# KlrShaK/opencv-SimpleSLAM

Hardware: AMD Instinct MI355X
Metric: frames/sec ALIKED+LightGlue @1241x376 (higher is better)
Workload: dtype f32 (contractions: f16 hi/lo split operands, f32 accumulate; 3 MFMA per product, 2 in attention's P.V = precision 'f16x3p1', the default since r05: profiles/r05_flip_soak.md, r06_flip_soak.md); 1 GPU; C2/C4: synthetic 1241x376x3 uint8 frame stream, ALIKED-n16 extract + LightGlue match (t-1,t), 2048 kpts/frame, min_conf 0.7, random-init weights; inputs resident in HBM before the timed region, features and matches left on the device (the `pcie` leg times the same pipeline with per-round H2D of the frames and D2H of {count, pairs}); max_kpts=2048, lightglue_layers_executed=9, pairs_per_lightglue_launch=8, frames_per_aliked_launch=8

## Files before the change

### opencv-simpleslam_amd/csrc/al_plan.hpp

```cpp
#pragma once
#include <algorithm>
#include <cstddef>
#include <cstdio>

namespace sslam {

constexpr int AL_LONG_SIDE = 1024;
constexpr int AL_PAD_DIV = 32;
constexpr int MAX_FRAMES = 16;
constexpr int B1_SW = 30;
constexpr int B2_SW = 30;
constexpr int DCN3_CS = 1;
constexpr int DCN4_CS = 4;
constexpr int AGG_PRE = 13;
constexpr int ST_W = 32, ST_H = 8;
constexpr int PRE_LDS_MAX = 48 * 1024;
constexpr int NHALO = 10;
constexpr int NW_R = 48, NW_OW = 64 - 2 * NHALO, NW_OH = NW_R - 2 * NHALO;
constexpr int HBINS = 4096;
constexpr int COLLECT_PPT = 16;
constexpr int SEL_CAP = 8192;
constexpr int EDGE_CAP = 2048;
constexpr int CAND_CAP = 1024 * 1024;
constexpr int REFINE_KPB = 32;
constexpr int SDDH_KSPLIT = 4;

constexpr int al_cdiv(int a, int b) { return (a + b - 1) / b; }

struct Dims {
    int H, W, C;
    int h, w;
    int Hp, Wp;
    int pl, pt;
};

enum class ALAggTile { T64x64, T64x128 };

struct ALPlan {
    int F, KF;
    int blur, ky, kx;
    float sy, sx;
    Dims d;
    int to_float_gx, pad_gx;
    int b1_strips, b1_nblk, b1_hs, b1_nb;
    int b2_strips, b2_nblk, b2_hs, b2_nb, b2_waves, b2_gx;
    int H2, W2, HW2, H3, W3, HW3, H4, W4, HW4;
    int pool3_gx, pool4_gx;
    int off3_gx, dcn3_gx, off4_gx, dcn4_gx;
// ... 82 lines not shown
enum class ALRefusal { None, Size, Frames, Blur };
inline ALRefusal al_refusal(const ALPlan& p, int Hp_cap, int Wp_cap, int max_frames, char* msg, size_t n) {
    const Dims& d = p.d;
    if (!(d.Hp <= Hp_cap && d.Wp <= Wp_cap && d.h >= 8 && d.w >= 8)) {
        snprintf(msg, n, "sslam_aliked: network size %dx%d outside the instance capacity %dx%d", d.Hp, d.Wp, Hp_cap, Wp_cap);
        return ALRefusal::Size;
    }
    if (!(p.F >= 1 && p.F <= max_frames)) {
        snprintf(msg, n, "sslam_aliked: %d frames, instance capacity %d", p.F, max_frames);
        return ALRefusal::Frames;
    }
    if (!(p.kx <= 31 && p.ky <= 31)) {
        snprintf(msg, n, "sslam_aliked: blur kernel too large (%d,%d)", p.kx, p.ky);
        return ALRefusal::Blur;
    }
    return ALRefusal::None;
}

struct ALKptPlan {
    int NK;
    int refine_gx, patch_gx, offsets_gx, sample_gx, finalize_gx;
    int rows_x16, rows64, rows64_x16;
    size_t plane;
};

inline ALKptPlan al_kpt_plan(int NK) {
    ALKptPlan k{};
    k.NK = NK;
    k.refine_gx = al_cdiv(NK, REFINE_KPB);
    k.patch_gx = al_cdiv(NK * 3, 4);
    k.rows64 = al_cdiv(NK, 64);
    k.offsets_gx = al_cdiv(NK * 32, 256);
    k.sample_gx = al_cdiv(NK * 16, 4);
    k.rows_x16 = NK * 16;
    k.rows64_x16 = al_cdiv(NK * 16, 64);
    k.finalize_gx = al_cdiv(NK, 4);
    k.plane = (size_t)(NK * 16 + 64) * 128;
    return k;
}

struct ALExtents {
    size_t ctrl, in_u8, fsrc, img, x1, x2, p3, off, t3, x3, p3cl, t3cl, p4cl, t4cl, p4, t4, x4, g2, g3, g4, g2cl, g3cl, g4cl;
    size_t s8, rnorm, g1cl, pre2, pre3, pre4, score, nms, bsum, cand, hist, kp_index, sel_keys;
    size_t kp_norm, kp_score, patch, h32, pos, sampled, feats, raw, out_xy, out_desc, out_score, out_n;
};

inline ALExtents al_extents(size_t HWp, size_t HWi, size_t NK) {
    ALExtents e{};
    e.ctrl = 1;
    e.in_u8 = HWi * 4;
    e.fsrc = 3 * HWi; e.img = 3 * HWp;
    e.x1 = 16 * HWp; e.x2 = 32 * HWp / 4;
    e.p3 = 32 * HWp / 64; e.off = 18 * HWp / 64;
    e.t3 = 64 * HWp / 64; e.x3 = 64 * HWp / 64;
    e.p3cl = 32 * HWp / 64; e.t3cl = 64 * HWp / 64;
    e.p4cl = 64 * HWp / 1024; e.t4cl = 128 * HWp / 1024;
    e.p4 = 64 * HWp / 1024; e.t4 = 128 * HWp / 1024; e.x4 = 128 * HWp / 1024;
    e.g2 = 32 * HWp / 4; e.g3 = 32 * HWp / 64; e.g4 = 32 * HWp / 1024;
    e.g2cl = 32 * HWp / 4; e.g3cl = 32 * HWp / 64; e.g4cl = 32 * HWp / 1024;
    e.s8 = 8 * HWp; e.rnorm = HWp; e.g1cl = 32 * HWp;
// ... 15 lines not shown
```

### opencv-simpleslam_amd/csrc/aliked_kernels.hip

```cpp
#include "common.hpp"
#include "al_plan.hpp"
#include "gemm_f32.hpp"
#include <type_traits>
#include "gemm_f16x3.hpp"

namespace {

using sslam::f32x16;
using sslam::acc_row;
using sslam::GemmSmem;
using sslam::GemmA;
using sslam::gemm_mainloop;
using sslam::Dims;
using sslam::MAX_FRAMES; using sslam::B1_SW; using sslam::B2_SW; using sslam::DCN3_CS; using sslam::DCN4_CS; using sslam::AGG_PRE;
using sslam::ST_W; using sslam::ST_H; using sslam::NHALO; using sslam::NW_R; using sslam::NW_OW; using sslam::NW_OH; using sslam::HBINS;
using sslam::COLLECT_PPT; using sslam::SEL_CAP; using sslam::EDGE_CAP; using sslam::REFINE_KPB; using sslam::SDDH_KSPLIT;

constexpr float SELU_SCALE = 1.0507009873554804934193349852946f;
constexpr float SELU_ALPHA = 1.6732632423543772848170429916717f;
__device__ __forceinline__ float selu(float x) {
    return SELU_SCALE * (x > 0.0f ? x : SELU_ALPHA * (__expf(x) - 1.0f));
}

__device__ __forceinline__ float selu_precise(float x) {
    return SELU_SCALE * (x > 0.0f ? x : SELU_ALPHA * expm1f(x));
}

struct ALCtrl {
    int n_cand;
    int n_kp;
    int overflow;
    int found;
    int range_overflow;
    int pad[11];
};

__device__ __forceinline__ void al_range_note(float amax, ALCtrl* ctrl) {
    if (amax >= 65520.0f && amax < INFINITY) ctrl->range_overflow = 1;
}
// ... 834 lines not shown
    float sy2, sx2, sy8, sx8, sy32, sx32;
    const float *g2cl, *g3cl, *g4cl;
    const float *pre2, *pre3, *pre4;
};

__device__ __forceinline__ Pyr pyr_at(Pyr P, int f, size_t fs) {
    P.x1 = fsh(P.x1, f, fs); P.g2 = fsh(P.g2, f, fs); P.g3 = fsh(P.g3, f, fs); P.g4 = fsh(P.g4, f, fs);
    P.g1cl = fsh(P.g1cl, f, fs); P.g2cl = fsh(P.g2cl, f, fs); P.g3cl = fsh(P.g3cl, f, fs); P.g4cl = fsh(P.g4cl, f, fs);
    P.pre2 = fsh(P.pre2, f, fs); P.pre3 = fsh(P.pre3, f, fs); P.pre4 = fsh(P.pre4, f, fs);
    return P;
}

struct UpTap { int o00, o01, o10, o11; float w00, w01, w10, w11; };

__device__ __forceinline__ UpTap up_tap(int y, int x, int Hp, int Wp, int S, float sy, float sx) {
    const int ih = Hp / S, iw = Wp / S;
    const float fy = sy * (float)y, fx = sx * (float)x;
    const int y0 = (int)fy, x0 = (int)fx;
    const int y1 = y0 + (y0 < ih - 1), x1 = x0 + (x0 < iw - 1);
    const float ly = fy - (float)y0, lx = fx - (float)x0, hy = 1.0f - ly, hx = 1.0f - lx;
    UpTap t;
    t.o00 = y0 * iw + x0; t.o01 = y0 * iw + x1; t.o10 = y1 * iw + x0; t.o11 = y1 * iw + x1;
    t.w00 = hx; t.w01 = lx; t.w10 = hy; t.w11 = ly;
    return t;
}
__device__ __forceinline__ float up_eval_cl(const float* __restrict__ p, const UpTap& t, int c) {
    return t.w10 * (t.w00 * p[t.o00 * 32 + c] + t.w01 * p[t.o01 * 32 + c]) +
           t.w11 * (t.w00 * p[t.o10 * 32 + c] + t.w01 * p[t.o11 * 32 + c]);
}
__device__ __forceinline__ float up_eval(const float* __restrict__ p, const UpTap& t) {
    return t.w10 * (t.w00 * p[t.o00] + t.w01 * p[t.o01]) + t.w11 * (t.w00 * p[t.o10] + t.w01 * p[t.o11]);
}

constexpr int PRE_UNROLL = 32;
__global__ __launch_bounds__(256) void al_agg_pre_kernel(const float* __restrict__ g2cl , const float* __restrict__ g3cl,
                                                         const float* __restrict__ g4cl, const float* __restrict__ ws0 ,
                                                         float* __restrict__ pre2, float* __restrict__ pre3, float* __restrict__ pre4,
                                                         int Hp, int Wp, size_t fs) {
    const int f = blockIdx.y;
    const int n2 = (Hp / 2) * (Wp / 2), n3 = (Hp / 8) * (Wp / 8), n4 = (Hp / 32) * (Wp / 32);
    int i = blockIdx.x * blockDim.x + threadIdx.x;
    const float* g; float* pre; int S, lvl;
    if (i < n2) { g = g2cl; pre = pre2; S = 2; lvl = 1; }
    else if (i < n2 + n3) { i -= n2; g = g3cl; pre = pre3; S = 8; lvl = 2; }
    else if (i < n2 + n3 + n4) { i -= n2 + n3; g = g4cl; pre = pre4; S = 32; lvl = 3; }
    else return;
// ... 608 lines not shown
    rnorm = fsh(rnorm, blockIdx.y, fs); kp_norm = fsh(kp_norm, blockIdx.y, fs); patch = fsh(patch, blockIdx.y, fs);
    ctrl = fsh(ctrl, blockIdx.y, fs);
    const int lane = threadIdx.x & 63, gw = blockIdx.x * 4 + __builtin_amdgcn_readfirstlane(threadIdx.x >> 6);
    const int n = gw / 3, trow = gw % 3;
    if (n >= ctrl->n_kp) return;
    const float kx = (kp_norm[2 * n] / 2.0f + 0.5f) * (float)(w - 1);
    const float ky = (kp_norm[2 * n + 1] / 2.0f + 0.5f) * (float)(h - 1);
    int cx = (int)((float)(int)kx - 1.5f + 1.0f), cy = (int)((float)(int)ky - 1.5f + 1.0f);
    cx = min(max(cx, 0), w - 1 - 3);
    cy = min(max(cy, 0), h - 1 - 3);
    float2 f[3];
#pragma unroll
    for (int tc = 0; tc < 3; ++tc) f[tc] = feat_pair32(P, rnorm, pl, pt, cy + trow, cx + tc, lane);
    const int c = lane & 31;
    const int ca = lane < 32 ? c : 32 + c, cb = lane < 32 ? 64 + c : 96 + c;
    float* dst = patch + (size_t)n * 1152;
#pragma unroll
    for (int tc = 0; tc < 3; ++tc) {
        dst[ca * 9 + 3 * trow + tc] = f[tc].x;
        dst[cb * 9 + 3 * trow + tc] = f[tc].y;
    }
}


__global__ void al_offsets_kernel(const float* __restrict__ h32 ,
                                  int cap, const float* __restrict__ b1,
                                  const float* __restrict__ w2 , const float* __restrict__ b2,
                                  const float* __restrict__ kp_norm, int h, int w, float max_off,
                                  float* __restrict__ pos , const ALCtrl* __restrict__ ctrl, size_t fs) {
    h32 = fsh(h32, blockIdx.y, fs); kp_norm = fsh(kp_norm, blockIdx.y, fs); pos = fsh(pos, blockIdx.y, fs); ctrl = fsh(ctrl, blockIdx.y, fs);
    const int i = blockIdx.x * blockDim.x + threadIdx.x;
    const int n = i / 32, o = i % 32;
    if (n >= ctrl->n_kp) return;
    float acc = 0.0f;
#pragma unroll 8
    for (int k = 0; k < 32; ++k) {
        float hv = b1[k];
#pragma unroll
        for (int z = 0; z < SDDH_KSPLIT; ++z) hv += h32[((size_t)z * cap + n) * 32 + k];
        acc = fmaf(selu(hv), w2[o * 32 + k], acc);
    }
    acc = fminf(fmaxf(acc + b2[o], -max_off), max_off);
    const int p = o & 15, comp = o >> 4;
    const float k0 = (kp_norm[2 * n + comp] / 2.0f + 0.5f) * (float)((comp ? h : w) - 1);
    pos[(n * 16 + p) * 2 + comp] = k0 + acc;
}

__global__ __launch_bounds__(256) void al_sample_kernel(Pyr P0, const float* __restrict__ rnorm, int pl, int pt,
                                                        int h, int w, const float* __restrict__ pos,
                                                        _Float16* __restrict__ sampled ,
                                                        size_t lo_off, ALCtrl* ctrl, size_t fs) {
    const Pyr P = pyr_at(P0, blockIdx.y, fs);
    rnorm = fsh(rnorm, blockIdx.y, fs); pos = fsh(pos, blockIdx.y, fs); sampled = fsh(sampled, blockIdx.y, fs); ctrl = fsh(ctrl, blockIdx.y, fs);
    const int lane = threadIdx.x & 63, gw = blockIdx.x * 4 + __builtin_amdgcn_readfirstlane(threadIdx.x >> 6);
    if (gw >= ctrl->n_kp * 16) return;
    const float gx = 2.0f * pos[gw * 2] / (float)(w - 1) - 1.0f, gy = 2.0f * pos[gw * 2 + 1] / (float)(h - 1) - 1.0f;
    const float ix = (gx + 1.0f) / 2.0f * (float)(w - 1), iy = (gy + 1.0f) / 2.0f * (float)(h - 1);
    const float fx = floorf(ix), fy = floorf(iy);
    const int x0 = (int)fx, y0 = (int)fy;
    const float wx1 = ix - fx, wy1 = iy - fy, wx0 = 1.0f - wx1, wy0 = 1.0f - wy1;
    float2 f[4]; float wgt[4];
    unsigned pixq[4]; UpTap t2[4], t3[4], t4[4];
#pragma unroll
    for (int q = 0; q < 4; ++q) {
        const int yy = y0 + (q >> 1), xx = x0 + (q & 1);
        const bool inside = yy >= 0 && yy < h && xx >= 0 && xx < w;
        wgt[q] = inside ? ((q & 1) ? wx1 : wx0) * ((q >> 1) ? wy1 : wy0) : 0.0f;
        const int yp = min(max(yy, 0), h - 1) + pt, xp = min(max(xx, 0), w - 1) + pl;
// ... 24 lines not shown
    if (lane < 32) {
#pragma unroll
        for (int q = 0; q < 4; ++q) aq[q] = at_b(P.g1cl, pixq[q] * 128u + cbo);
        level_shared(P.g3cl, t3, bq);
    } else {
#pragma unroll
        for (int q = 0; q < 4; ++q) aq[q] = up_eval_cl32(P.g2cl, t2[q], cbo);
        level_shared(P.g4cl, t4, bq);
    }
#pragma unroll
    for (int q = 0; q < 4; ++q) { const float r = rnorm[pixq[q]]; f[q] = make_float2(aq[q] * r, bq[q] * r); }
    float ax = 0.0f, bx = 0.0f;
#pragma unroll
    for (int q = 0; q < 4; ++q) { ax = fmaf(f[q].x, wgt[q], ax); bx = fmaf(f[q].y, wgt[q], bx); }
    const int c = lane & 31;
    const int ca = lane < 32 ? c : 32 + c, cb = lane < 32 ? 64 + c : 96 + c;
    unsigned h2, l2; float amax = 0.0f;
    sslam::split2_fast(ax, bx, h2, l2, amax);
    al_range_note(amax, ctrl);
    const _Float16 hv[2] = {__builtin_bit_cast(sslam::half2v, h2)[0], __builtin_bit_cast(sslam::half2v, h2)[1]};
    const _Float16 lv[2] = {__builtin_bit_cast(sslam::half2v, l2)[0], __builtin_bit_cast(sslam::half2v, l2)[1]};
    sampled[(size_t)gw * 128 + ca] = hv[0]; sampled[(size_t)gw * 128 + cb] = hv[1];
    sampled[lo_off + (size_t)gw * 128 + ca] = lv[0]; sampled[lo_off + (size_t)gw * 128 + cb] = lv[1];
}

template <int BM, int BN, int TM, int TN>
__global__ __launch_bounds__(256) void al_gemm_kernel(const float* __restrict__ A, int K, const float* __restrict__ Wt,
                                                      const float* __restrict__ bias, int N, float* __restrict__ C,
                                                      int rows_per_kp, int row_cap, int do_selu,
                                                      const ALCtrl* __restrict__ ctrl, int KS, size_t fs) {
    __shared__ GemmSmem<BM, BN> sm;
    const int zs = blockIdx.z % KS, fr = blockIdx.z / KS;
    A = fsh(A, fr, fs); C = fsh(C, fr, fs); ctrl = fsh(ctrl, fr, fs);
    const int M = ctrl->n_kp * rows_per_kp;
    const int row0 = blockIdx.y * BM, col0 = blockIdx.x * BN;
    if (row0 >= M) return;
    const int kper = K / KS, koff = zs * kper;
    C += (size_t)zs * row_cap * N;
    GemmA ga{A + koff, K, A + koff, K, kper};
    f32x16 acc[TM][TN];
    gemm_mainloop<BM, BN, TM, TN>(ga, Wt + koff, K, kper, row0, row_cap, col0, N, sm, acc);
    const int lane = threadIdx.x & 63, wave = threadIdx.x >> 6, wm = wave >> 1, wn = wave & 1;
#pragma unroll
    for (int i = 0; i < TM; ++i)
#pragma unroll
        for (int j = 0; j < TN; ++j) {
            const int col = col0 + wn * 32 * TN + j * 32 + (lane & 31);
            const float b = (bias && col < N) ? bias[col] : 0.0f;
#pragma unroll
            for (int r = 0; r < 16; ++r) {
                const int row = row0 + wm * 32 * TM + i * 32 + acc_row(r, lane);
                float v = acc[i][j][r] + b;
                if (do_selu) v = selu(v);
                if (row < M && col < N) C[(size_t)row * N + col] = v;
            }
        }
}

template <int BM, int BN, int TM, int TN, bool SPLIT_OUT>
__global__ __launch_bounds__(256) void al_gemm_h_kernel(const _Float16* __restrict__ A, size_t a_lo, int K,
                                                        const _Float16* __restrict__ W, size_t w_lo, int N,
                                                        float* __restrict__ C, _Float16* __restrict__ Ch, size_t c_lo,
                                                        int rows_per_kp, int row_cap, ALCtrl* ctrl, int KS,
                                                        size_t fs) {
    __shared__ sslam::GemmSmemH<BM, BN> sm;
    const int zs = blockIdx.z % KS, fr = blockIdx.z / KS;
    A = fsh(A, fr, fs); C = fsh(C, fr, fs); Ch = fsh(Ch, fr, fs); ctrl = fsh(ctrl, fr, fs);
    const int M = ctrl->n_kp * rows_per_kp;
    const int row0 = blockIdx.y * BM, col0 = blockIdx.x * BN;
    if (row0 >= M) return;
    const int kper = K / KS, koff = zs * kper;
    sslam::GemmAH ga{{A + koff, A + a_lo + koff}, {A + koff, A + a_lo + koff}, K, kper};
    f32x16 c1[TM][TN], c2[TM][TN];
    sslam::gemm_mainloop_h<BM, BN, TM, TN>(ga, sslam::SplitPtr{W + koff, W + w_lo + koff}, K, kper, row0, row_cap, col0, N, sm, c1, c2);
    const int lane = threadIdx.x & 63, wave = threadIdx.x >> 6, wm = wave >> 1, wn = wave & 1;
    if constexpr (!SPLIT_OUT) C += (size_t)zs * row_cap * N;
    float amax = 0.0f;
#pragma unroll
    for (int i = 0; i < TM; ++i)
#pragma unroll
        for (int j = 0; j < TN; ++j) {
            const int col = col0 + wn * 32 * TN + j * 32 + (lane & 31);
#pragma unroll
            for (int r = 0; r < 16; ++r) {
                const int row = row0 + wm * 32 * TM + i * 32 + acc_row(r, lane);
                float v = c1[i][j][r] + c2[i][j][r] * sslam::SPLIT_INV;
                if (row >= M || col >= N) continue;
                if constexpr (SPLIT_OUT) {
                    v = selu(v);
                    const float aa = fabsf(v);
                    amax = fmaxf(amax, aa);
                    const _Float16 hi = aa < 6.103515625e-5f ? (_Float16)0.0f : (_Float16)v;
                    Ch[(size_t)row * N + col] = hi;
                    Ch[c_lo + (size_t)row * N + col] = (_Float16)((v - (float)hi) * sslam::SPLIT_SCALE);
                } else {
                    C[(size_t)row * N + col] = v;
                }
            }
        }
    if constexpr (SPLIT_OUT) al_range_note(amax, ctrl);
}

__global__ void al_split_kernel(const float* __restrict__ src, _Float16* __restrict__ dst, size_t n, int* range_flag) {
    const size_t i = (size_t)blockIdx.x * blockDim.x + threadIdx.x;
    if (i >= n) return;
    _Float16 hi, lo;
    al_split_weight(src[i], hi, lo, range_flag);
    dst[i] = hi;
    dst[n + i] = lo;
}

__global__ __launch_bounds__(256) void al_finalize_kernel(const float* __restrict__ raw , int cap,
                                                          const float* __restrict__ kp_norm,
                                                          const float* __restrict__ kp_score, int h, int w, float scale_x,
                                                          float scale_y, FrameOut outs, const ALCtrl* __restrict__ ctrl,
                                                          int* range_sticky, size_t fs) {
    raw = fsh(raw, blockIdx.y, fs); kp_norm = fsh(kp_norm, blockIdx.y, fs); kp_score = fsh(kp_score, blockIdx.y, fs);
    ctrl = fsh(ctrl, blockIdx.y, fs);
    float* __restrict__ xy_out = outs.xy[blockIdx.y]; float* __restrict__ desc_out = outs.desc[blockIdx.y];
    float* __restrict__ score_out = outs.score[blockIdx.y]; int32_t* __restrict__ n_out = outs.n[blockIdx.y];
    const int lane = threadIdx.x & 63, n = blockIdx.x * 4 + (threadIdx.x >> 6);
    if (blockIdx.x == 0 && threadIdx.x == 0) {
        n_out[0] = ctrl->range_overflow ? -1 : ctrl->n_kp;
// ... 75 lines not shown

int al_bind_weights(sslam_aliked* g, size_t n_floats) {
    size_t off = 0;
    auto take = [&](size_t n) { const float* p = g->blob + off; off += al_pad64(n); return p; };
    auto conv = [&](int ci, int co) { ALConvW c; c.w = take((size_t)ci * 9 * co); c.a = take(co); c.b = take(co); return c; };
    auto dcn = [&](int ci, int co) {
        ALDcnW c; c.ow = take((size_t)ci * 9 * 18); c.ob = take(18); c.w = take((size_t)ci * 9 * co);
        c.a = take(co); c.b = take(co); return c;
    };
    g->b1c1 = conv(3, 16); g->b1c2 = conv(16, 16);
    g->b2c1 = conv(16, 32); g->b2c2 = conv(32, 32); g->b2dw = take(16 * 32); g->b2db = take(32);
    g->b3c1 = dcn(32, 64); g->b3c2 = dcn(64, 64); g->b3dw = take(32 * 64); g->b3db = take(64);
    g->b4c1 = dcn(64, 128); g->b4c2 = dcn(128, 128); g->b4dw = take(64 * 128); g->b4db = take(128);
    g->gw1 = take(16 * 32); g->gw2 = take(32 * 32); g->gw3 = take(64 * 32); g->gw4 = take(128 * 32);
    g->sh0 = take(128 * 8); g->sh2 = take(8 * 9 * 4); g->sh4 = take(4 * 9 * 4); g->sh6 = take(4 * 9);
    g->d_ow = take(32 * 1152); g->d_ob = take(32); g->d_w2 = take(32 * 32); g->d_b2 = take(32);
    g->d_sf = take(128 * 128); g->d_agg = take((size_t)128 * 2048);
    SSLAM_REQUIRE(off == n_floats, "sslam_aliked_create: weight blob has %zu floats, expected %zu", n_floats, off);
    return 0;
}

constexpr int SEL_LDS = (SEL_CAP + EDGE_CAP) * 8;

int al_enqueue(sslam_aliked* g, const sslam::ALPlan& p, const FrameIn& srcs, int n_limit, const FrameOut& outs) {
    hipStream_t s = g->ctx->stream;
    (void)hipGetLastError();
    const Dims& d = p.d;
    const sslam::ALKptPlan& k = g->kp;
    const int F = p.F, KF = p.KF, NK = k.NK;
    const size_t fs = g->fs;
    const dim3 b256(256);
    hipLaunchKernelGGL(al_reset_kernel, dim3(F), b256, 0, s, g->ctrl, g->hist, fs, g->gk, p.kx, p.sx, p.ky, p.sy);

    hipLaunchKernelGGL(al_preprocess_kernel, dim3(p.pre_gx, p.pre_gy, F), b256, (size_t)p.pre_lds, s, srcs, g->img, d, g->gk, p.kx, p.ky,
                       p.blur, PreTile{p.pre_tw, p.pre_th, p.pre_cols, p.pre_rows, p.pre_raw}, fs);
    hipLaunchKernelGGL(al_block1_rows_kernel, dim3(p.b1_strips, p.b1_nb, F), dim3(64), 0, s, g->img, g->x1, d.Hp, d.Wp, p.b1_hs,
                       g->b1c1.w, g->b1c1.a, g->b1c1.b, g->b1c2f, g->b1c2.a, g->b1c2.b, g->ctrl, fs);
    hipLaunchKernelGGL(al_block2_rows_kernel, dim3(p.b2_gx), b256, B2_LDS, s, g->x1, g->x2, p.H2, p.W2, p.b2_hs, p.b2_nb, p.b2_strips,
                       p.b2_waves, g->b2c1f, g->b2c2f, g->b2c1.a, g->b2c1.b, g->b2db, g->b2c2.a, g->b2c2.b, g->ctrl, fs);
    const dim3 off3 = dim3(p.off3_gx, p.H3, F), dcn3 = dim3(p.dcn3_gx, p.H3, F);
    hipLaunchKernelGGL(al_avgpool_kernel, dim3(p.pool3_gx, F), b256, 0, s, g->x2, g->p3, 32, p.H2, p.W2, 4, fs, g->p3cl);
    hipLaunchKernelGGL((al_offset_conv_h_kernel<32>), off3, b256, 0, s, g->p3cl, g->off, p.H3, p.W3, g->b3c1of, g->b3c1.ob, p.mo3, g->ctrl, fs);
    hipLaunchKernelGGL((al_dcn_h_kernel<32, 64, 0, DCN3_CS>), dcn3, b256, 0, s, g->p3cl, g->off, nullptr, p.H3, p.W3, g->b3c1f, g->b3c1.b, nullptr, g->t3, g->t3cl, g->ctrl, fs);
    hipLaunchKernelGGL((al_offset_conv_h_kernel<64>), off3, b256, 0, s, g->t3cl, g->off, p.H3, p.W3, g->b3c2of, g->b3c2.ob, p.mo3, g->ctrl, fs);
    hipLaunchKernelGGL((al_dcn_h_kernel<64, 64, 32, DCN3_CS>), dcn3, b256, 0, s, g->t3cl, g->off, g->p3cl, p.H3, p.W3, g->b3c2f, g->b3c2.b, g->b3db, g->x3, nullptr, g->ctrl, fs);
    const dim3 off4 = dim3(p.off4_gx, p.H4, F), dcn4 = dim3(p.dcn4_gx, p.H4, F);
    sslam::graph_cut(s);
    hipLaunchKernelGGL(al_avgpool_kernel, dim3(p.pool4_gx, F), b256, 0, s, g->x3, g->p4, 64, p.H3, p.W3, 4, fs, g->p4cl);
    hipLaunchKernelGGL((al_offset_conv_h_kernel<64>), off4, b256, 0, s, g->p4cl, g->off, p.H4, p.W4, g->b4c1of, g->b4c1.ob, p.mo4, g->ctrl, fs);
    hipLaunchKernelGGL((al_dcn_h_kernel<64, 128, 0, DCN4_CS>), dcn4, b256, 0, s, g->p4cl, g->off, nullptr, p.H4, p.W4, g->b4c1f, g->b4c1.b, nullptr, g->t4, g->t4cl, g->ctrl, fs);
    hipLaunchKernelGGL((al_offset_conv_h_kernel<128>), off4, b256, 0, s, g->t4cl, g->off, p.H4, p.W4, g->b4c2of, g->b4c2.ob, p.mo4, g->ctrl, fs);
    hipLaunchKernelGGL((al_dcn_h_kernel<128, 128, 64, DCN4_CS>), dcn4, b256, 0, s, g->t4cl, g->off, g->p4cl, p.H4, p.W4, g->b4c2f, g->b4c2.b, g->b4db, g->x4, nullptr, g->ctrl, fs);
    hipLaunchKernelGGL(al_gate_kernel<32>, dim3(p.gate2_gx, F), b256, 0, s, g->x2, g->g2, p.HW2, g->gw2, g->g2cl, fs);
    hipLaunchKernelGGL(al_gate_small_kernel, dim3(p.gate34_gx, F), b256, 0, s, GateSmall{g->x3, g->g3, 64, p.HW3, g->gw3, g->g3cl},
                       GateSmall{g->x4, g->g4, 128, p.HW4, g->gw4, g->g4cl}, p.gate3_gx, fs);
    Pyr P{g->x1, g->g2, g->g3, g->g4, g->gw1, d.Hp, d.Wp, g->g1cl};
    P.sy2 = p.sy2; P.sx2 = p.sx2; P.sy8 = p.sy8; P.sx8 = p.sx8; P.sy32 = p.sy32; P.sx32 = p.sx32;
    P.g2cl = g->g2cl; P.g3cl = g->g3cl; P.g4cl = g->g4cl;
    P.pre2 = g->pre2; P.pre3 = g->pre3; P.pre4 = g->pre4;
    hipLaunchKernelGGL(al_agg_pre_kernel, dim3(p.agg_pre_gx, F), b256, 0, s, g->g2, g->g3, g->g4, g->sh0, g->pre2, g->pre3, g->pre4,
                       d.Hp, d.Wp, fs);
    hipLaunchKernelGGL(al_aggregate_kernel, dim3(p.pad_gx, d.Hp, F), b256, 0, s, P, g->sh0, g->s8, g->rnorm, fs);
    hipLaunchKernelGGL(al_score_tail_kernel, dim3(p.tail_gx, p.tail_gy, F), dim3(ST_T), 0, s, g->s8, d.Hp, d.Wp, g->sh2, g->sh4, g->sh6,
                       g->score, d.h, d.w, d.pl, d.pt, fs);
    hipLaunchKernelGGL(al_nms_wave_kernel, dim3(p.nms_gx, F), b256, 0, s, g->score, d.h, d.w, p.nbx, p.n_tiles, g->nms, g->bsum, 0.2f,
                       g->cand, g->cand_cap, g->ctrl, g->hist, fs);
    sslam::graph_cut(s);
    hipLaunchKernelGGL(al_collect_kernel, dim3(p.collect_gx, F), b256, 0, s, g->nms, p.npx, 0.0f, 1, g->bsum, p.n_tiles, g->cand,
                       g->cand_cap, g->ctrl, g->hist, fs);
    hipLaunchKernelGGL(al_select_kernel, dim3(F), dim3(1024), SEL_LDS, s, g->cand, g->cand_cap, n_limit, g->sel_keys, g->ctrl, g->hist, fs);
    hipLaunchKernelGGL(al_refine_kernel, dim3(k.refine_gx, F), b256, 0, s, g->score, d.h, d.w, g->sel_keys, g->kp_index, g->kp_norm,
                       g->kp_score, g->ctrl, fs);
    hipLaunchKernelGGL(al_patch_kernel, dim3(k.patch_gx, F), b256, 0, s, P, g->rnorm, d.pl, d.pt, d.h, d.w, g->kp_norm, g->patch, g->ctrl, fs);
    hipLaunchKernelGGL((al_gemm_kernel<64, 64, 1, 1>), dim3(1, k.rows64, KF), b256, 0, s, g->patch, 1152, g->d_ow, nullptr, 32, g->h32,
                       1, NK, 0, g->ctrl, SDDH_KSPLIT, fs);
    hipLaunchKernelGGL(al_offsets_kernel, dim3(k.offsets_gx, F), b256, 0, s, g->h32, NK, g->d_ob, g->d_w2, g->d_b2, g->kp_norm, d.h, d.w,
                       p.mo, g->pos, g->ctrl, fs);
    _Float16* sampled_h = reinterpret_cast<_Float16*>(g->sampled);
    _Float16* feats_h = reinterpret_cast<_Float16*>(g->feats);
    hipLaunchKernelGGL(al_sample_kernel, dim3(k.sample_gx, F), b256, 0, s, P, g->rnorm, d.pl, d.pt, d.h, d.w, g->pos, sampled_h,
                       k.plane, g->ctrl, fs);
    hipLaunchKernelGGL((al_gemm_h_kernel<64, 128, 1, 2, true>), dim3(1, k.rows64_x16, F), b256, 0, s, sampled_h, k.plane, 128, g->d_sf_s,
                       (size_t)128 * 128, 128, nullptr, feats_h, k.plane, 16, k.rows_x16, g->ctrl, 1, fs);
    if (p.agg_tile == sslam::ALAggTile::T64x128)
        hipLaunchKernelGGL((al_gemm_h_kernel<64, 128, 1, 2, false>), dim3(1, k.rows64, KF), b256, 0, s, feats_h, k.plane, 2048,
                           g->d_agg_s, (size_t)128 * 2048, 128, g->raw, nullptr, 0, 1, NK, g->ctrl, SDDH_KSPLIT, fs);
    else
        hipLaunchKernelGGL((al_gemm_h_kernel<64, 64, 1, 1, false>), dim3(2, k.rows64, KF), b256, 0, s, feats_h, k.plane, 2048,
                           g->d_agg_s, (size_t)128 * 2048, 128, g->raw, nullptr, 0, 1, NK, g->ctrl, SDDH_KSPLIT, fs);
    hipLaunchKernelGGL(al_finalize_kernel, dim3(k.finalize_gx, F), b256, 0, s, g->raw, NK, g->kp_norm, g->kp_score, d.h, d.w,
                       p.scale_x, p.scale_y, outs, g->ctrl, g->range_sticky, fs);
    SSLAM_HIP_CHECK(hipGetLastError());
    return 0;
}

struct Frames { FrameIn in{}; FrameOut out{}; };
Frames al_one_frame(const uint8_t* img_dev, float* xy_out, float* desc_out, float* score_out, int32_t* n_out) {
    Frames f;
    f.in.img[0] = img_dev; f.out.xy[0] = xy_out; f.out.desc[0] = desc_out; f.out.score[0] = score_out; f.out.n[0] = n_out;
    return f;
// ... 80 lines not shown
        hipStream_t s = ctx->stream;
        SSLAM_HIP_CHECK(hipMemsetAsync(g->range_sticky, 0, 4 * sizeof(int), s));
        hipLaunchKernelGGL(al_conv32_wfrag_kernel, dim3(sslam::cdiv(32 * 288, 256)), dim3(256), 0, s, g->b2c2.w, g->b2c2f, g->range_sticky);
        hipLaunchKernelGGL(al_conv16_wfrag_kernel, dim3(sslam::cdiv(5 * 64 * 8, 256)), dim3(256), 0, s, g->b1c2.w, g->b1c2f, g->range_sticky);
        hipLaunchKernelGGL(al_conv32p_wfrag_kernel, dim3(sslam::cdiv(10 * 64 * 8, 256)), dim3(256), 0, s, g->b2c1.w, g->b2dw, g->b2c1f, g->range_sticky);
        hipLaunchKernelGGL(al_split_kernel, dim3(sslam::cdiv(128 * 128, 256)), dim3(256), 0, s, g->d_sf, g->d_sf_s, (size_t)128 * 128, g->range_sticky);
        hipLaunchKernelGGL(al_split_kernel, dim3(sslam::cdiv(128 * 2048, 256)), dim3(256), 0, s, g->d_agg, g->d_agg_s, (size_t)128 * 2048, g->range_sticky);
        hipLaunchKernelGGL((al_dcn_wfrag_kernel<32, 64, 0>), dim3(sslam::cdiv((9 * 2 + 0) * 2 * 512, 256)), dim3(256), 0, s, g->b3c1.w, g->b3c1.a, nullptr, g->b3c1f, g->range_sticky);
        hipLaunchKernelGGL((al_dcn_wfrag_kernel<64, 64, 32>), dim3(sslam::cdiv((9 * 4 + 2) * 2 * 512, 256)), dim3(256), 0, s, g->b3c2.w, g->b3c2.a, g->b3dw, g->b3c2f, g->range_sticky);
        hipLaunchKernelGGL((al_dcn_wfrag_kernel<64, 128, 0>), dim3(sslam::cdiv((9 * 4 + 0) * 4 * 512, 256)), dim3(256), 0, s, g->b4c1.w, g->b4c1.a, nullptr, g->b4c1f, g->range_sticky);
        hipLaunchKernelGGL((al_dcn_wfrag_kernel<128, 128, 64>), dim3(sslam::cdiv((9 * 8 + 4) * 4 * 512, 256)), dim3(256), 0, s, g->b4c2.w, g->b4c2.a, g->b4dw, g->b4c2f, g->range_sticky);
        hipLaunchKernelGGL(al_offc_wfrag_kernel<32>, dim3(sslam::cdiv(18 * 512, 256)), dim3(256), 0, s, g->b3c1.ow, g->b3c1of, g->range_sticky);
        hipLaunchKernelGGL(al_offc_wfrag_kernel<64>, dim3(sslam::cdiv(36 * 512, 256)), dim3(256), 0, s, g->b3c2.ow, g->b3c2of, g->range_sticky);
        hipLaunchKernelGGL(al_offc_wfrag_kernel<64>, dim3(sslam::cdiv(36 * 512, 256)), dim3(256), 0, s, g->b4c1.ow, g->b4c1of, g->range_sticky);
        hipLaunchKernelGGL(al_offc_wfrag_kernel<128>, dim3(sslam::cdiv(72 * 512, 256)), dim3(256), 0, s, g->b4c2.ow, g->b4c2of, g->range_sticky);
        int wflag = 0;
        SSLAM_HIP_CHECK(hipMemcpyAsync(&wflag, g->range_sticky, sizeof(int), hipMemcpyDeviceToHost, s));
        SSLAM_HIP_CHECK(hipStreamSynchronize(s));
        SSLAM_REQUIRE(!wflag, "sslam_aliked_create: a weight (BN scale folded) with |value| >= 65520 does not fit the fp16 planes "
                              "of the split-precision stages");
    }
    SSLAM_HIP_CHECK(hipFuncSetAttribute((const void*)al_block2_rows_kernel, hipFuncAttributeMaxDynamicSharedMemorySize, (int)B2_LDS));
    SSLAM_HIP_CHECK(hipFuncSetAttribute((const void*)al_select_kernel, hipFuncAttributeMaxDynamicSharedMemorySize, SEL_LDS));
    sslam::ctx_retain(ctx);
    *out = g.release();
    return 0;
}

int sslam_aliked_create(sslam_ctx* ctx, const float* weights, size_t n_floats, int max_h, int max_w,
                        int max_kpts, sslam_aliked** out) {
    return sslam_aliked_create_batched(ctx, weights, n_floats, max_h, max_w, max_kpts, 1, out);
}

int sslam_aliked_destroy(sslam_aliked* g) {
    return sslam::destroy_instance(g);
}

static int al_check_image(sslam_aliked* g, int H, int W, int C, int max_kpts) {
    SSLAM_REQUIRE(C == 1 || C == 3 || C == 4, "sslam_aliked_extract: %d channels (want 1 gray, 3 BGR or 4 BGRA)", C);
    SSLAM_REQUIRE(H >= 16 && W >= 16 && H <= g->max_h && W <= g->max_w,
                  "sslam_aliked_extract: image %dx%d outside the instance capacity %dx%d", W, H, g->max_w, g->max_h);
    SSLAM_REQUIRE(max_kpts >= 1 && max_kpts <= g->max_kpts, "sslam_aliked_extract: max_kpts %d exceeds capacity %d",
                  max_kpts, g->max_kpts);
    return 0;
}

// ... 101 lines not shown
            dims[0] = d.h; dims[1] = d.w; dims[2] = d.Hp; dims[3] = d.Wp; dims[4] = d.pl; dims[5] = d.pt;
            dims[6] = c.n_cand; dims[7] = c.n_kp;
            SSLAM_REQUIRE(bytes <= sizeof(dims), "sslam_aliked_debug_read: dims is 32 bytes");
            memcpy(dst, dims, bytes);
            return 0;
        }
        case 3: src = g->x1; cap = e.x1 * 4; break;
        case 4: src = g->x2; cap = e.x2 * 4; break;
        case 5: src = g->x3; cap = e.x3 * 4; break;
        case 6: src = g->x4; cap = e.x4 * 4; break;
        case 7: src = g->img; cap = e.img * 4; break;
        case 8: src = g->nms; cap = (size_t)d.h * d.w * 4; break;
        case 9: src = g->kp_norm; cap = (size_t)g->max_kpts * 8; break;
        case 10: src = g->g1cl; cap = e.g1cl * 4; break;
        case 11: src = g->rnorm; cap = e.rnorm * 4; break;
        case 12: src = g->g2; cap = e.g2 * 4; break;
        case 13: src = g->g3; cap = e.g3 * 4; break;
        case 14: src = g->g4; cap = e.g4 * 4; break;
        case 15: src = g->pre2; cap = e.pre2 * 4; break;
        case 16: src = g->pre3; cap = e.pre3 * 4; break;
        case 17: src = g->pre4; cap = e.pre4 * 4; break;
        case 18: src = g->s8; cap = e.s8 * 4; break;
        case 19: src = g->pos; cap = (size_t)g->max_kpts * 32 * 4; break;
        case 20: src = g->patch; cap = (size_t)g->max_kpts * 1152 * 4; break;
        default: SSLAM_REQUIRE(false, "sslam_aliked_debug_read: unknown buffer %d", which);
    }
    SSLAM_REQUIRE(bytes <= cap, "sslam_aliked_debug_read: %zu bytes requested, buffer has %zu", bytes, cap);
    SSLAM_HIP_CHECK(hipMemcpy(dst, src, bytes, hipMemcpyDeviceToHost));
    return 0;
}

}
```

Measured before the change: 1262 frames/s.

## Fuse ALIKED offset patch gather, GEMM and MLP tail into one kernel

Replaces the patch-gather, split-K offset GEMM and offsets MLP kernels with a single kernel. It builds each keypoint's 3x3 upsampled patch directly in LDS, runs the MFMA contraction with one wave per k-slice, and reduces and applies the second layer in place. This removes two launches and the global round-trip of the patch and h32 buffers, at the cost of heavy LDS use and scattered gathers inside the kernel. The SPLIT_OUT GEMM epilogue is also changed to stage the tile in LDS and write vectorised half8 stores. The patch kernel is now run only from the debug-read path.

After: 1270 frames/s, median of 6. Within noise of the previous version (+0.7%).

```diff
diff --git a/opencv-simpleslam_amd/csrc/al_plan.hpp b/opencv-simpleslam_amd/csrc/al_plan.hpp
--- a/opencv-simpleslam_amd/csrc/al_plan.hpp
+++ b/opencv-simpleslam_amd/csrc/al_plan.hpp
@@ -24,6 +24,7 @@
 constexpr int CAND_CAP = 1024 * 1024;
 constexpr int REFINE_KPB = 32;
 constexpr int SDDH_KSPLIT = 4;
+constexpr int OFFS_ROWS = 32;
 
 constexpr int al_cdiv(int a, int b) { return (a + b - 1) / b; }
 
@@ -152,6 +153,7 @@
     int refine_gx, patch_gx, offsets_gx, sample_gx, finalize_gx;
     int rows_x16, rows64, rows64_x16;
     size_t plane;
+    int fused_rows, fused_gx;
 };
 
 inline ALKptPlan al_kpt_plan(int NK) {
@@ -166,6 +168,8 @@
     k.rows64_x16 = al_cdiv(NK * 16, 64);
     k.finalize_gx = al_cdiv(NK, 4);
     k.plane = (size_t)(NK * 16 + 64) * 128;
+    k.fused_rows = OFFS_ROWS;
+    k.fused_gx = al_cdiv(NK, OFFS_ROWS);
     return k;
 }
 
diff --git a/opencv-simpleslam_amd/csrc/aliked_kernels.hip b/opencv-simpleslam_amd/csrc/aliked_kernels.hip
--- a/opencv-simpleslam_amd/csrc/aliked_kernels.hip
+++ b/opencv-simpleslam_amd/csrc/aliked_kernels.hip
@@ -8,13 +8,11 @@
 
 using sslam::f32x16;
 using sslam::acc_row;
-using sslam::GemmSmem;
-using sslam::GemmA;
-using sslam::gemm_mainloop;
+using sslam::mfma32;
 using sslam::Dims;
 using sslam::MAX_FRAMES; using sslam::B1_SW; using sslam::B2_SW; using sslam::DCN3_CS; using sslam::DCN4_CS; using sslam::AGG_PRE;
 using sslam::ST_W; using sslam::ST_H; using sslam::NHALO; using sslam::NW_R; using sslam::NW_OW; using sslam::NW_OH; using sslam::HBINS;
-using sslam::COLLECT_PPT; using sslam::SEL_CAP; using sslam::EDGE_CAP; using sslam::REFINE_KPB; using sslam::SDDH_KSPLIT;
+using sslam::COLLECT_PPT; using sslam::SEL_CAP; using sslam::EDGE_CAP; using sslam::REFINE_KPB; using sslam::SDDH_KSPLIT; using sslam::OFFS_ROWS;
 
 constexpr float SELU_SCALE = 1.0507009873554804934193349852946f;
 constexpr float SELU_ALPHA = 1.6732632423543772848170429916717f;
@@ -895,6 +893,18 @@
     UpTap t;
     t.o00 = y0 * iw + x0; t.o01 = y0 * iw + x1; t.o10 = y1 * iw + x0; t.o11 = y1 * iw + x1;
     t.w00 = hx; t.w01 = lx; t.w10 = hy; t.w11 = ly;
+    return t;
+}
+__device__ __forceinline__ UpTap up_tap_patch(int y, int x, int ih, int iw, float sy, float sx, bool fused) {
+    const float yf = (float)y, xf = (float)x;
+    const float fy = __fmul_rn(sy, yf), fx = __fmul_rn(sx, xf);
+    const int y0 = (int)fy, x0 = (int)fx;
+    const int y1 = y0 + (y0 < ih - 1), x1 = x0 + (x0 < iw - 1);
+    const float ly = fused ? fmaf(sy, yf, -(float)y0) : __fsub_rn(fy, (float)y0);
+    const float lx = fused ? fmaf(sx, xf, -(float)x0) : __fsub_rn(fx, (float)x0);
+    UpTap t;
+    t.o00 = y0 * iw + x0; t.o01 = y0 * iw + x1; t.o10 = y1 * iw + x0; t.o11 = y1 * iw + x1;
+    t.w00 = __fsub_rn(1.0f, lx); t.w01 = lx; t.w10 = __fsub_rn(1.0f, ly); t.w11 = ly;
     return t;
 }
 __device__ __forceinline__ float up_eval_cl(const float* __restrict__ p, const UpTap& t, int c) {
@@ -1549,28 +1559,136 @@
     }
 }
 
-
-__global__ void al_offsets_kernel(const float* __restrict__ h32 ,
-                                  int cap, const float* __restrict__ b1,
-                                  const float* __restrict__ w2 , const float* __restrict__ b2,
-                                  const float* __restrict__ kp_norm, int h, int w, float max_off,
-                                  float* __restrict__ pos , const ALCtrl* __restrict__ ctrl, size_t fs) {
-    h32 = fsh(h32, blockIdx.y, fs); kp_norm = fsh(kp_norm, blockIdx.y, fs); pos = fsh(pos, blockIdx.y, fs); ctrl = fsh(ctrl, blockIdx.y, fs);
-    const int i = blockIdx.x * blockDim.x + threadIdx.x;
-    const int n = i / 32, o = i % 32;
-    if (n >= ctrl->n_kp) return;
-    float acc = 0.0f;
+constexpr int OF_ROWS = OFFS_ROWS;
+constexpr int OF_CP = 16;
+constexpr int OF_KP = OF_CP * 9;
+constexpr int OF_LD = OF_KP + 4;
+constexpr int OF_TILE = OF_ROWS * OF_LD;
+constexpr int OF_PIX = OF_ROWS * 9 / 4;
+constexpr int OF_UN = 9;
+constexpr int OF_LDS = SDDH_KSPLIT * OF_TILE * 4;
+static_assert((OF_PIX / 2) % OF_UN == 0, "whole batches of pixels");
+static_assert(OF_KP % 8 == 0 && 32 % OF_CP == 0 && OF_LD % 4 == 0 && OF_PIX % 2 == 0, "whole groups of 8 k; 16-byte fragment reads");
+static_assert(OF_ROWS == 32 && OF_TILE >= 1024 + 33 * 32 && SDDH_KSPLIT == 4, "the tail's arrays fit a level tile; one wave per k-slice");
+
+AL_AGG_TARGET __global__ __launch_bounds__(256, 2) void al_offsets_fused_kernel(Pyr P0, const float* __restrict__ rnorm, int pl, int pt, int h, int w,
+                                                                  const float* __restrict__ kp_norm,
+                                                                  const float* __restrict__ ow ,
+                                                                  const float* __restrict__ b1, const float* __restrict__ w2 ,
+                                                                  const float* __restrict__ b2, float max_off,
+                                                                  float* __restrict__ pos , const ALCtrl* __restrict__ ctrl, size_t fs) {
+    extern __shared__ __attribute__((aligned(16))) float of_lds[];
+    const Pyr P = pyr_at(P0, blockIdx.y, fs);
+    rnorm = fsh(rnorm, blockIdx.y, fs); kp_norm = fsh(kp_norm, blockIdx.y, fs); pos = fsh(pos, blockIdx.y, fs); ctrl = fsh(ctrl, blockIdx.y, fs);
+    const int n_kp = ctrl->n_kp, row0 = blockIdx.x * OF_ROWS;
+    if (row0 >= n_kp) return;
+    const int t = threadIdx.x, lane = t & 63, wave = __builtin_amdgcn_readfirstlane(t >> 6);
+    __shared__ int corner[2 * OF_ROWS];
+    if (t < OF_ROWS) {
+        int cx = 0, cy = 0;
+        if (row0 + t < n_kp) {
+            const int n = row0 + t;
+            const float kx = (kp_norm[2 * n] / 2.0f + 0.5f) * (float)(w - 1);
+            const float ky = (kp_norm[2 * n + 1] / 2.0f + 0.5f) * (float)(h - 1);
+            cx = (int)((float)(int)kx - 1.5f + 1.0f); cy = (int)((float)(int)ky - 1.5f + 1.0f);
+            cx = min(max(cx, 0), w - 1 - 3);
+            cy = min(max(cy, 0), h - 1 - 3);
+        }
+        corner[2 * t] = cx; corner[2 * t + 1] = cy;
+    }
+    __syncthreads();
+
+    const int slot = (lane >> 4) & 1, upper = lane >> 5, cl = lane & 15;
+    const int hh = lane >> 5, lr = lane & 31;
+    float* tile_a = of_lds + upper * OF_TILE;
+    float* tile_b = of_lds + (2 + upper) * OF_TILE;
+    const float* base_a = upper ? P.g2cl : P.g1cl;
+    const float* base_b = upper ? P.g4cl : P.g3cl;
+    const int ih_a = P.Hp / 2, iw_a = P.Wp / 2, ih_b = upper ? P.Hp / 32 : P.Hp / 8, iw_b = upper ? P.Wp / 32 : P.Wp / 8;
+    const float sy_b = upper ? P.sy32 : P.sy8, sx_b = upper ? P.sx32 : P.sx8;
+    const float* frag_a = of_lds + wave * OF_TILE + lr * OF_LD + 4 * hh;
+    const float* frag_w = ow + (size_t)lr * 1152 + wave * 288 + 4 * hh;
+    f32x16 acc;
+#pragma unroll
+    for (int r = 0; r < 16; ++r) acc[r] = 0.0f;
+    for (int pass = 0; pass < 32 / OF_CP; ++pass) {
+        if (pass) __syncthreads();
+        const unsigned cb = 4u * (unsigned)(pass * OF_CP + cl);
+#pragma unroll 1
+        for (int bt = 0; bt < OF_PIX / 2 / OF_UN; ++bt) {
+            float va[OF_UN][4], vb[OF_UN][4], rn[OF_UN];
+            UpTap ta[OF_UN], tb[OF_UN];
+            int lo[OF_UN];
+#pragma unroll
+            for (int j = 0; j < OF_UN; ++j) {
+                const int q = wave * OF_PIX + 2 * (bt * OF_UN + j) + slot, rl = q / 9, tap = q - 9 * rl;
+                const int cx = corner[2 * rl], cy = corner[2 * rl + 1];
+                const int yp = cy + tap / 3 + pt, xp = cx + tap % 3 + pl;
+                const unsigned pix = (unsigned)(yp * P.Wp + xp);
+                ta[j] = up_tap_patch(yp, xp, ih_a, iw_a, P.sy2, P.sx2, true);
+                tb[j] = up_tap_patch(yp, xp, ih_b, iw_b, sy_b, sx_b, false);
+                va[j][0] = at_b(base_a, (upper ? (unsigned)ta[j].o00 : pix) * 128u + cb);
+                va[j][1] = at_b(base_a, (upper ? (unsigned)ta[j].o01 : pix) * 128u + cb);
+                va[j][2] = at_b(base_a, (upper ? (unsigned)ta[j].o10 : pix) * 128u + cb);
+                va[j][3] = at_b(base_a, (upper ? (unsigned)ta[j].o11 : pix) * 128u + cb);
+                vb[j][0] = at_b(base_b, (unsigned)tb[j].o00 * 128u + cb);
+                vb[j][1] = at_b(base_b, (unsigned)tb[j].o01 * 128u + cb);
+                vb[j][2] = at_b(base_b, (unsigned)tb[j].o10 * 128u + cb);
+                vb[j][3] = at_b(base_b, (unsigned)tb[j].o11 * 128u + cb);
+                rn[j] = rnorm[pix];
+                lo[j] = rl * OF_LD + cl * 9 + tap;
+            }
+#pragma unroll
+            for (int j = 0; j < OF_UN; ++j) {
+                const float a = upper ? up_mix(ta[j], va[j][0], va[j][1], va[j][2], va[j][3]) : va[j][0];
+                const float b = up_mix(tb[j], vb[j][0], vb[j][1], vb[j][2], vb[j][3]);
+                tile_a[lo[j]] = a * rn[j];
+                tile_b[lo[j]] = b * rn[j];
+            }
+        }
+        float4 wf[OF_KP / 8];
+#pragma unroll
+        for (int g = 0; g < OF_KP / 8; ++g) LD4(wf[g], frag_w + pass * OF_KP + g * 8);
+        __syncthreads();
+#pragma unroll
+        for (int g = 0; g < OF_KP / 8; ++g) {
+            float4 af;
+            LD4(af, frag_a + g * 8);
+            acc = mfma32(af.x, wf[g].x, acc);
+            acc = mfma32(af.y, wf[g].y, acc);
+            acc = mfma32(af.z, wf[g].z, acc);
+            acc = mfma32(af.w, wf[g].w, acc);
+        }
+    }
+    float* part = of_lds + wave * OF_TILE;
+#pragma unroll
+    for (int r = 0; r < 16; ++r) part[acc_row(r, lane) * 32 + lr] = acc[r] + 0.0f;
+    float* sel = of_lds + 1024;
+    float* w2s = of_lds + OF_TILE + 1024;
+    __syncthreads();
+#pragma unroll
+    for (int i = 0; i < 4; ++i) { const int e = t + 256 * i; w2s[(e >> 5) * 33 + (e & 31)] = w2[e]; }
+#pragma unroll
+    for (int i = 0; i < 4; ++i) {
+        const int e = t + 256 * i, k = e & 31;
+        float hv = b1[k];
+#pragma unroll
+        for (int z = 0; z < SDDH_KSPLIT; ++z) hv += of_lds[z * OF_TILE + e];
+        sel[(e >> 5) * 33 + k] = selu(hv);
+    }
+    __syncthreads();
+#pragma unroll
+    for (int i = 0; i < 4; ++i) {
+        const int e = t + 256 * i, rl = e >> 5, o = e & 31, n = row0 + rl;
+        float a = 0.0f;
 #pragma unroll 8
-    for (int k = 0; k < 32; ++k) {
-        float hv = b1[k];
-#pragma unroll
-        for (int z = 0; z < SDDH_KSPLIT; ++z) hv += h32[((size_t)z * cap + n) * 32 + k];
-        acc = fmaf(selu(hv), w2[o * 32 + k], acc);
-    }
-    acc = fminf(fmaxf(acc + b2[o], -max_off), max_off);
-    const int p = o & 15, comp = o >> 4;
-    const float k0 = (kp_norm[2 * n + comp] / 2.0f + 0.5f) * (float)((comp ? h : w) - 1);
-    pos[(n * 16 + p) * 2 + comp] = k0 + acc;
+        for (int k = 0; k < 32; ++k) a = fmaf(sel[rl * 33 + k], w2s[o * 33 + k], a);
+        if (n >= n_kp) continue;
+        a = fminf(fmaxf(a + b2[o], -max_off), max_off);
+        const int p = o & 15, comp = o >> 4;
+        const float k0 = (kp_norm[2 * n + comp] / 2.0f + 0.5f) * (float)((comp ? h : w) - 1);
+        pos[(n * 16 + p) * 2 + comp] = k0 + a;
+    }
 }
 
 __global__ __launch_bounds__(256) void al_sample_kernel(Pyr P0, const float* __restrict__ rnorm, int pl, int pt,
@@ -1641,39 +1759,6 @@
     const _Float16 lv[2] = {__builtin_bit_cast(sslam::half2v, l2)[0], __builtin_bit_cast(sslam::half2v, l2)[1]};
     sampled[(size_t)gw * 128 + ca] = hv[0]; sampled[(size_t)gw * 128 + cb] = hv[1];
     sampled[lo_off + (size_t)gw * 128 + ca] = lv[0]; sampled[lo_off + (size_t)gw * 128 + cb] = lv[1];
-}
-
-template <int BM, int BN, int TM, int TN>
-__global__ __launch_bounds__(256) void al_gemm_kernel(const float* __restrict__ A, int K, const float* __restrict__ Wt,
-                                                      const float* __restrict__ bias, int N, float* __restrict__ C,
-                                                      int rows_per_kp, int row_cap, int do_selu,
-                                                      const ALCtrl* __restrict__ ctrl, int KS, size_t fs) {
-    __shared__ GemmSmem<BM, BN> sm;
-    const int zs = blockIdx.z % KS, fr = blockIdx.z / KS;
-    A = fsh(A, fr, fs); C = fsh(C, fr, fs); ctrl = fsh(ctrl, fr, fs);
-    const int M = ctrl->n_kp * rows_per_kp;
-    const int row0 = blockIdx.y * BM, col0 = blockIdx.x * BN;
-    if (row0 >= M) return;
-    const int kper = K / KS, koff = zs * kper;
-    C += (size_t)zs * row_cap * N;
-    GemmA ga{A + koff, K, A + koff, K, kper};
-    f32x16 acc[TM][TN];
-    gemm_mainloop<BM, BN, TM, TN>(ga, Wt + koff, K, kper, row0, row_cap, col0, N, sm, acc);
-    const int lane = threadIdx.x & 63, wave = threadIdx.x >> 6, wm = wave >> 1, wn = wave & 1;
-#pragma unroll
-    for (int i = 0; i < TM; ++i)
-#pragma unroll
-        for (int j = 0; j < TN; ++j) {
-            const int col = col0 + wn * 32 * TN + j * 32 + (lane & 31);
-            const float b = (bias && col < N) ? bias[col] : 0.0f;
-#pragma unroll
-            for (int r = 0; r < 16; ++r) {
-                const int row = row0 + wm * 32 * TM + i * 32 + acc_row(r, lane);
-                float v = acc[i][j][r] + b;
-                if (do_selu) v = selu(v);
-                if (row < M && col < N) C[(size_t)row * N + col] = v;
-            }
-        }
 }
 
 template <int BM, int BN, int TM, int TN, bool SPLIT_OUT>
@@ -1693,31 +1778,61 @@
     f32x16 c1[TM][TN], c2[TM][TN];
     sslam::gemm_mainloop_h<BM, BN, TM, TN>(ga, sslam::SplitPtr{W + koff, W + w_lo + koff}, K, kper, row0, row_cap, col0, N, sm, c1, c2);
     const int lane = threadIdx.x & 63, wave = threadIdx.x >> 6, wm = wave >> 1, wn = wave & 1;
-    if constexpr (!SPLIT_OUT) C += (size_t)zs * row_cap * N;
-    float amax = 0.0f;
-#pragma unroll
-    for (int i = 0; i < TM; ++i)
-#pragma unroll
-        for (int j = 0; j < TN; ++j) {
-            const int col = col0 + wn * 32 * TN + j * 32 + (lane & 31);
-#pragma unroll
-            for (int r = 0; r < 16; ++r) {
-                const int row = row0 + wm * 32 * TM + i * 32 + acc_row(r, lane);
-                float v = c1[i][j][r] + c2[i][j][r] * sslam::SPLIT_INV;
-                if (row >= M || col >= N) continue;
-                if constexpr (SPLIT_OUT) {
-                    v = selu(v);
-                    const float aa = fabsf(v);
-                    amax = fmaxf(amax, aa);
-                    const _Float16 hi = aa < 6.103515625e-5f ? (_Float16)0.0f : (_Float16)v;
-                    Ch[(size_t)row * N + col] = hi;
-                    Ch[c_lo + (size_t)row * N + col] = (_Float16)((v - (float)hi) * sslam::SPLIT_SCALE);
-                } else {
+    if constexpr (SPLIT_OUT) {
+        constexpr int ELD = BN + 4;
+        constexpr int CH = BN / 8, ITERS = BM * CH / 256;
+        static_assert(sizeof(sm) >= (size_t)BM * ELD * 4 && (BM * CH) % 256 == 0, "the staged tile fits the operand ring");
+        float* epi = reinterpret_cast<float*>(&sm);
+#pragma unroll
+        for (int i = 0; i < TM; ++i)
+#pragma unroll
+            for (int j = 0; j < TN; ++j) {
+                const int cl = wn * 32 * TN + j * 32 + (lane & 31);
+#pragma unroll
+                for (int r = 0; r < 16; ++r) {
+                    const int rl = wm * 32 * TM + i * 32 + acc_row(r, lane);
+                    epi[rl * ELD + cl] = selu(c1[i][j][r] + c2[i][j][r] * sslam::SPLIT_INV);
+                }
+            }
+        __syncthreads();
+        float amax = 0.0f;
+#pragma unroll
+        for (int it = 0; it < ITERS; ++it) {
+            const int u = threadIdx.x + it * 256, rl = u / CH, cl = (u % CH) * 8;
+            const int row = row0 + rl, col = col0 + cl;
+            if (row >= M || col >= N) continue;
+            const float4 a = *reinterpret_cast<const float4*>(&epi[rl * ELD + cl]);
+            const float4 b = *reinterpret_cast<const float4*>(&epi[rl * ELD + cl + 4]);
+            const float v8[8] = {a.x, a.y, a.z, a.w, b.x, b.y, b.z, b.w};
+            sslam::half8 h8, l8;
+#pragma unroll
+            for (int e = 0; e < 8; ++e) {
+                const float v = v8[e], aa = fabsf(v);
+                amax = fmaxf(amax, aa);
+                const _Float16 hi = aa < 6.103515625e-5f ? (_Float16)0.0f : (_Float16)v;
+                h8[e] = hi;
+                l8[e] = (_Float16)((v - (float)hi) * sslam::SPLIT_SCALE);
+            }
+            *reinterpret_cast<sslam::half8*>(Ch + (size_t)row * N + col) = h8;
+            *reinterpret_cast<sslam::half8*>(Ch + c_lo + (size_t)row * N + col) = l8;
+        }
+        al_range_note(amax, ctrl);
+    } else {
+        C += (size_t)zs * row_cap * N;
+#pragma unroll
+        for (int i = 0; i < TM; ++i)
+#pragma unroll
+            for (int j = 0; j < TN; ++j) {
+                const int col = col0 + wn * 32 * TN + j * 32 + (lane & 31);
+#pragma unroll
+                for (int r = 0; r < 16; ++r) {
+                    const int row = row0 + wm * 32 * TM + i * 32 + acc_row(r, lane);
+                    const float v = c1[i][j][r] + c2[i][j][r] * sslam::SPLIT_INV;
+                    if (row >= M || col >= N) continue;
                     C[(size_t)row * N + col] = v;
                 }
             }
-        }
-    if constexpr (SPLIT_OUT) al_range_note(amax, ctrl);
+    }
 }
 
 __global__ void al_split_kernel(const float* __restrict__ src, _Float16* __restrict__ dst, size_t n, int* range_flag) {
@@ -1839,6 +1954,14 @@
 
 constexpr int SEL_LDS = (SEL_CAP + EDGE_CAP) * 8;
 
+Pyr al_pyr(const sslam_aliked* g, const sslam::ALPlan& p) {
+    Pyr P{g->x1, g->g2, g->g3, g->g4, g->gw1, p.d.Hp, p.d.Wp, g->g1cl};
+    P.sy2 = p.sy2; P.sx2 = p.sx2; P.sy8 = p.sy8; P.sx8 = p.sx8; P.sy32 = p.sy32; P.sx32 = p.sx32;
+    P.g2cl = g->g2cl; P.g3cl = g->g3cl; P.g4cl = g->g4cl;
+    P.pre2 = g->pre2; P.pre3 = g->pre3; P.pre4 = g->pre4;
+    return P;
+}
+
 int al_enqueue(sslam_aliked* g, const sslam::ALPlan& p, const FrameIn& srcs, int n_limit, const FrameOut& outs) {
     hipStream_t s = g->ctx->stream;
     (void)hipGetLastError();
@@ -1871,10 +1994,7 @@
     hipLaunchKernelGGL(al_gate_kernel<32>, dim3(p.gate2_gx, F), b256, 0, s, g->x2, g->g2, p.HW2, g->gw2, g->g2cl, fs);
     hipLaunchKernelGGL(al_gate_small_kernel, dim3(p.gate34_gx, F), b256, 0, s, GateSmall{g->x3, g->g3, 64, p.HW3, g->gw3, g->g3cl},
                        GateSmall{g->x4, g->g4, 128, p.HW4, g->gw4, g->g4cl}, p.gate3_gx, fs);
-    Pyr P{g->x1, g->g2, g->g3, g->g4, g->gw1, d.Hp, d.Wp, g->g1cl};
-    P.sy2 = p.sy2; P.sx2 = p.sx2; P.sy8 = p.sy8; P.sx8 = p.sx8; P.sy32 = p.sy32; P.sx32 = p.sx32;
-    P.g2cl = g->g2cl; P.g3cl = g->g3cl; P.g4cl = g->g4cl;
-    P.pre2 = g->pre2; P.pre3 = g->pre3; P.pre4 = g->pre4;
+    const Pyr P = al_pyr(g, p);
     hipLaunchKernelGGL(al_agg_pre_kernel, dim3(p.agg_pre_gx, F), b256, 0, s, g->g2, g->g3, g->g4, g->sh0, g->pre2, g->pre3, g->pre4,
                        d.Hp, d.Wp, fs);
     hipLaunchKernelGGL(al_aggregate_kernel, dim3(p.pad_gx, d.Hp, F), b256, 0, s, P, g->sh0, g->s8, g->rnorm, fs);
@@ -1888,11 +2008,8 @@
     hipLaunchKernelGGL(al_select_kernel, dim3(F), dim3(1024), SEL_LDS, s, g->cand, g->cand_cap, n_limit, g->sel_keys, g->ctrl, g->hist, fs);
     hipLaunchKernelGGL(al_refine_kernel, dim3(k.refine_gx, F), b256, 0, s, g->score, d.h, d.w, g->sel_keys, g->kp_index, g->kp_norm,
                        g->kp_score, g->ctrl, fs);
-    hipLaunchKernelGGL(al_patch_kernel, dim3(k.patch_gx, F), b256, 0, s, P, g->rnorm, d.pl, d.pt, d.h, d.w, g->kp_norm, g->patch, g->ctrl, fs);
-    hipLaunchKernelGGL((al_gemm_kernel<64, 64, 1, 1>), dim3(1, k.rows64, KF), b256, 0, s, g->patch, 1152, g->d_ow, nullptr, 32, g->h32,
-                       1, NK, 0, g->ctrl, SDDH_KSPLIT, fs);
-    hipLaunchKernelGGL(al_offsets_kernel, dim3(k.offsets_gx, F), b256, 0, s, g->h32, NK, g->d_ob, g->d_w2, g->d_b2, g->kp_norm, d.h, d.w,
-                       p.mo, g->pos, g->ctrl, fs);
+    hipLaunchKernelGGL(al_offsets_fused_kernel, dim3(k.fused_gx, F), b256, OF_LDS, s, P, g->rnorm, d.pl, d.pt, d.h, d.w, g->kp_norm,
+                       g->d_ow, g->d_ob, g->d_w2, g->d_b2, p.mo, g->pos, g->ctrl, fs);
     _Float16* sampled_h = reinterpret_cast<_Float16*>(g->sampled);
     _Float16* feats_h = reinterpret_cast<_Float16*>(g->feats);
     hipLaunchKernelGGL(al_sample_kernel, dim3(k.sample_gx, F), b256, 0, s, P, g->rnorm, d.pl, d.pt, d.h, d.w, g->pos, sampled_h,
@@ -2019,6 +2136,7 @@
     }
     SSLAM_HIP_CHECK(hipFuncSetAttribute((const void*)al_block2_rows_kernel, hipFuncAttributeMaxDynamicSharedMemorySize, (int)B2_LDS));
     SSLAM_HIP_CHECK(hipFuncSetAttribute((const void*)al_select_kernel, hipFuncAttributeMaxDynamicSharedMemorySize, SEL_LDS));
+    SSLAM_HIP_CHECK(hipFuncSetAttribute((const void*)al_offsets_fused_kernel, hipFuncAttributeMaxDynamicSharedMemorySize, OF_LDS));
     sslam::ctx_retain(ctx);
     *out = g.release();
     return 0;
@@ -2166,7 +2284,17 @@
         case 17: src = g->pre4; cap = e.pre4 * 4; break;
         case 18: src = g->s8; cap = e.s8 * 4; break;
         case 19: src = g->pos; cap = (size_t)g->max_kpts * 32 * 4; break;
-        case 20: src = g->patch; cap = (size_t)g->max_kpts * 1152 * 4; break;
+        case 20: {
+            char why[160];
+            const sslam::ALPlan p = sslam::al_plan(std::max(d.H, 1), std::max(d.W, 1), d.C, 1);
+            if (d.Hp > 0 && sslam::al_refusal(p, g->Hp_cap, g->Wp_cap, g->max_frames, why, sizeof(why)) == sslam::ALRefusal::None) {
+                hipLaunchKernelGGL(al_patch_kernel, dim3(g->kp.patch_gx, 1), dim3(256), 0, g->ctx->stream, al_pyr(g, p), g->rnorm, d.pl,
+                                   d.pt, d.h, d.w, g->kp_norm, g->patch, g->ctrl, g->fs);
+                SSLAM_HIP_CHECK(hipGetLastError());
+                SSLAM_HIP_CHECK(hipStreamSynchronize(g->ctx->stream));
+            }
+            src = g->patch; cap = (size_t)g->max_kpts * 1152 * 4; break;
+        }
         default: SSLAM_REQUIRE(false, "sslam_aliked_debug_read: unknown buffer %d", which);
     }
     SSLAM_REQUIRE(bytes <= cap, "sslam_aliked_debug_read: %zu bytes requested, buffer has %zu", bytes, cap);
```
